# TennisBowling/grandine

Measured on AMD Instinct MI355X. Metric: verified BLS signature sets/sec (whole node), higher is better.
Workload: dtype u32 (exact 381-bit Montgomery: 12 x 32-bit limbs; 14 x 28-bit limbs in the Miller products and the square-root exponentiations); 1 GPU; C2: 16 independent batches of 4096 single-pubkey sets per GPU per step, each its own random-scalar multi_verify (segments of one submission); config=C2, streams_in_flight=2, parallelism=1 GPU

## Files before the change

grandine_amd/csrc/bls_dfp_tables.h:

```cpp
#pragma once
#include <stdint.h>
namespace gbls { namespace dfp {
constexpr uint64_t X_ABS = 0xd201000000010000ull;
constexpr int W12D_ZERO = 72, W12D_NSLOT = 73;
__constant__ uint8_t W12D_PRE[54][8] = {
  {0, 12, 12, 12, 12, 12, 12, 12},
  {1, 12, 12, 12, 12, 12, 12, 12},
  {0, 1, 12, 12, 12, 12, 12, 12},
  {2, 12, 12, 12, 12, 12, 12, 12},
  {3, 12, 12, 12, 12, 12, 12, 12},
  {2, 3, 12, 12, 12, 12, 12, 12},
  {4, 12, 12, 12, 12, 12, 12, 12},
  {5, 12, 12, 12, 12, 12, 12, 12},
  {4, 5, 12, 12, 12, 12, 12, 12},
  {2, 4, 12, 12, 12, 12, 12, 12},
  {3, 5, 12, 12, 12, 12, 12, 12},
  {2, 3, 4, 5, 12, 12, 12, 12},
  {0, 2, 12, 12, 12, 12, 12, 12},
  {1, 3, 12, 12, 12, 12, 12, 12},
  {0, 1, 2, 3, 12, 12, 12, 12},
  {0, 4, 12, 12, 12, 12, 12, 12},
  {1, 5, 12, 12, 12, 12, 12, 12},
  {0, 1, 4, 5, 12, 12, 12, 12},
  {6, 12, 12, 12, 12, 12, 12, 12},
// ... 266 lines not shown
};
__constant__ uint32_t K_FROB2[6][16] = {
  {0xdba9366u, 0xb7fde37u, 0x25bc342u, 0x894e275u, 0x1e97784u, 0x9dc1f5bu, 0x2b2b91bu, 0xfcafb87u, 0x06f497du, 0xa9b0bb2u, 0x137cc89u, 0xe399594u, 0xd9d20d7u, 0x000411cu, 0x0000000u, 0x0000000u},
  {0x9f59d6au, 0xdf5d035u, 0x06879dbu, 0x20871fdu, 0x40009cbu, 0xafc0735u, 0xb30b1b0u, 0x540793cu, 0xe51b64cu, 0xbe10100u, 0xc7f3381u, 0xc5133bcu, 0x9a653e5u, 0x00126bau, 0x0000000u, 0x0000000u},
  {0xc3b0a04u, 0x275f1fdu, 0xe0cb699u, 0x9738f87u, 0x2169246u, 0x11fe7dau, 0x87df895u, 0x5757db5u, 0xde26cceu, 0x145f54eu, 0xb4766f8u, 0xe179e28u, 0xc09330du, 0x000e59du, 0x0000000u, 0x0000000u},
  {0x2451745u, 0x47021c8u, 0x1a43c77u, 0x76b08a0u, 0x43aa727u, 0x0334bb4u, 0xcb477b7u, 0xf6d55a4u, 0x4080206u, 0xa1fc1c4u, 0xa6fe9b9u, 0x0300f1du, 0x44d18a8u, 0x0015ef4u, 0x0000000u, 0x0000000u},
  {0x60a0d41u, 0x1fa2fcau, 0x39785deu, 0xdf77918u, 0x22414e0u, 0xf1363dau, 0x4367f21u, 0x9f7d7efu, 0x6259538u, 0x8d9cc75u, 0xf2882c1u, 0x21870f4u, 0x843e59au, 0x0007956u, 0x0000000u, 0x0000000u},
  {0x3c4a0a7u, 0xd7a0e02u, 0x5f34920u, 0x68c5b8du, 0x40d8c65u, 0x8ef8335u, 0x6e9383du, 0x9c2d376u, 0x694deb6u, 0x374d827u, 0x0604f4bu, 0x0520689u, 0x5e10672u, 0x000ba73u, 0x0000000u, 0x0000000u},
};
constexpr uint32_t K_P_U[16] = {0xfffaaabu, 0xfefffffu, 0x3ffffb9u, 0xfffeb15u, 0x6241eabu, 0xa0f6b0fu, 0xf6730d2u, 0xf38512bu, 0x4774b84u, 0x4bacd76u, 0xba7b643u, 0xe69a4b1u, 0x1ea397fu, 0x001a011u, 0x0000000u, 0x0000000u};
constexpr uint32_t K_PINV_U[16] = {0xffcfffdu, 0xf3fffcfu, 0x113e889u, 0xdb92d9du, 0xb48286au, 0xf0c8e30u, 0xc16ef2eu, 0x8eb2db4u, 0x9ecca0eu, 0x68cf581u, 0x316fee2u, 0xfc9468bu, 0x106feaau, 0xa0ceb06u, 0x27f7e27u, 0xd0d7f87u};
__constant__ uint32_t K_P[16] = {0x0fffaaabu, 0x0fefffffu, 0x03ffffb9u, 0x0fffeb15u, 0x06241eabu, 0x0a0f6b0fu, 0x0f6730d2u, 0x0f38512bu, 0x04774b84u, 0x04bacd76u, 0x0ba7b643u, 0x0e69a4b1u, 0x01ea397fu, 0x0001a011u, 0x00000000u, 0x00000000u};
__constant__ uint32_t K_CIN[16] = {0x062b6c9du, 0x07d3988au, 0x0aff4e96u, 0x0383fa8eu, 0x08464532u, 0x08703310u, 0x0f823830u, 0x0d396d7cu, 0x05efebb5u, 0x04e16bc1u, 0x07cd07eeu, 0x056c4fabu, 0x0d3a884eu, 0x00002cb5u, 0x00000000u, 0x00000000u};
__constant__ uint32_t K_COUT[16] = {0x0002fffdu, 0x00900000u, 0x0c000276u, 0x0000bc40u, 0x08baebf4u, 0x05753c75u, 0x055f4898u, 0x07052574u, 0x07ce5853u, 0x056ec6d7u, 0x071a97a2u, 0x0e4935c0u, 0x0ec3fa80u, 0x00015f65u, 0x00000000u, 0x00000000u};
__constant__ uint32_t K_ONE[16] = {0x0dba9366u, 0x0b7fde37u, 0x025bc342u, 0x0894e275u, 0x01e97784u, 0x09dc1f5bu, 0x02b2b91bu, 0x0fcafb87u, 0x006f497du, 0x0a9b0bb2u, 0x0137cc89u, 0x0e399594u, 0x0d9d20d7u, 0x0000411cu, 0x00000000u, 0x00000000u};
__constant__ uint32_t K_BIAS_R1[16] = {0x7ffd5558u, 0x7f7ffff8u, 0x7ffffdc8u, 0x7fff58a2u, 0x7120f558u, 0x707b5874u, 0x7b39868eu, 0x79c28958u, 0x73ba5c20u, 0x75d66babu, 0x7d3db213u, 0x734d2586u, 0x7f51cbf8u, 0x000d0081u, 0x00000000u, 0x00000000u};
__constant__ uint32_t K_BIAS_R2[16] = {0x3ff55560u, 0x3dfffffcu, 0x3ffff73cu, 0x3ffd62a4u, 0x3483d57cu, 0x31ed61e9u, 0x3ce61a51u, 0x370a257bu, 0x3ee9709bu, 0x3759aec5u, 0x34f6c866u, 0x3d349634u, 0x3d472ff9u, 0x00340220u, 0x00000000u, 0x00000000u};
__constant__ uint32_t K_BIAS_NEG[16] = {0x2fd55580u, 0x27fffffdu, 0x2fffdcfdu, 0x2ff58a9du, 0x220f55fdu, 0x27b587afu, 0x2398694eu, 0x2c2895f9u, 0x2ba5c277u, 0x2d66bb21u, 0x23db21a3u, 0x24d258dbu, 0x251cbff1u, 0x00d0088du, 0x00000000u, 0x00000000u};
__constant__ uint32_t K_BIAS_SQ[16] = {0x5eaaac00u, 0x5ffffffau, 0x5ffee7f6u, 0x5fac54fau, 0x507aaffau, 0x5dac3d84u, 0x5cc34a7eu, 0x5144afd4u, 0x5d2e13c9u, 0x5b35d918u, 0x5ed90d29u, 0x5692c6e4u, 0x58e5ff95u, 0x06804475u, 0x00000000u, 0x00000000u};
__constant__ uint32_t K_BIAS_GY[16] = {0x3f555600u, 0x3ffffffcu, 0x3fff73fau, 0x3fd62a7cu, 0x383d57fcu, 0x3ed61ec1u, 0x3e61a53eu, 0x30a257e9u, 0x3e9709e4u, 0x359aec8bu, 0x3f6c8694u, 0x33496371u, 0x3472ffcau, 0x0340223au, 0x00000000u, 0x00000000u};
__constant__ uint32_t K_BIAS_GS[16] = {0x4eaaac00u, 0x4ffffffbu, 0x4ffee7f7u, 0x4fac54fbu, 0x407aaffbu, 0x4dac3d85u, 0x4cc34a7fu, 0x4144afd5u, 0x4d2e13cau, 0x4b35d919u, 0x4ed90d2au, 0x4692c6e5u, 0x48e5ff96u, 0x06804476u, 0x00000000u, 0x00000000u};
__constant__ uint32_t K_INVFIX[16] = {0x06b0f5bau, 0x079ca4b9u, 0x0d0e7df7u, 0x02e27c00u, 0x0b969102u, 0x005b1d88u, 0x0f3b945du, 0x0051805fu, 0x02710831u, 0x0ea54e57u, 0x095e4bd3u, 0x055e4a8du, 0x042b7a0fu, 0x0000e87du, 0x00000000u, 0x00000000u};
__constant__ uint32_t K_PSI_CX1[16] = {0x03c4a0a7u, 0x0d7a0e02u, 0x05f34920u, 0x068c5b8du, 0x040d8c65u, 0x08ef8335u, 0x06e9383du, 0x09c2d376u, 0x0694deb6u, 0x0374d827u, 0x00604f4bu, 0x00520689u, 0x05e10672u, 0x0000ba73u, 0x00000000u, 0x00000000u};
__constant__ uint32_t K_PSI_CY0[16] = {0x04c22d67u, 0x0947f37bu, 0x0853ec71u, 0x002485e1u, 0x015b9b2au, 0x0b1268c5u, 0x0b62e6e6u, 0x045fb220u, 0x04dd1ca9u, 0x04fcbb2cu, 0x00af4fc4u, 0x05fd3770u, 0x0475233bu, 0x0000faafu, 0x00000000u, 0x00000000u};
__constant__ uint32_t K_PSI_CY1[16] = {0x0b3d7d44u, 0x06a80c84u, 0x0bac1348u, 0x0fdb6533u, 0x04c88381u, 0x0efd024au, 0x040449ebu, 0x0ad89f0bu, 0x0f9a2edbu, 0x0fbe1249u, 0x0af8667eu, 0x086c6d41u, 0x0d751644u, 0x0000a561u, 0x00000000u, 0x00000000u};
__constant__ uint32_t K_PSI2_CX[16] = {0x060a0d41u, 0x01fa2fcau, 0x039785deu, 0x0df77918u, 0x022414e0u, 0x0f1363dau, 0x04367f21u, 0x09f7d7efu, 0x06259538u, 0x08d9cc75u, 0x0f2882c1u, 0x021870f4u, 0x0843e59au, 0x00007956u, 0x00000000u, 0x00000000u};
__constant__ uint32_t K_PSI2_CY[16] = {0x02451745u, 0x047021c8u, 0x01a43c77u, 0x076b08a0u, 0x043aa727u, 0x00334bb4u, 0x0cb477b7u, 0x0f6d55a4u, 0x04080206u, 0x0a1fc1c4u, 0x0a6fe9b9u, 0x00300f1du, 0x044d18a8u, 0x00015ef4u, 0x00000000u, 0x00000000u};
__constant__ uint32_t K_BIASK[10][16] = {
  {0x2fff5556u, 0x2fdffffdu, 0x27ffff71u, 0x2fffd628u, 0x2c483d55u, 0x241ed61cu, 0x2ece61a3u, 0x2e70a255u, 0x28ee9707u, 0x29759aeau, 0x274f6c84u, 0x2cd34961u, 0x23d472fdu, 0x00034020u, 0x00000000u, 0x00000000u},
  {0x2ffeaaacu, 0x2fbffffdu, 0x2ffffee5u, 0x2fffac52u, 0x28907aadu, 0x283dac3bu, 0x2d9cc348u, 0x2ce144adu, 0x21dd2e11u, 0x22eb35d7u, 0x2e9ed90bu, 0x29a692c4u, 0x27a8e5fdu, 0x00068042u, 0x00000000u, 0x00000000u},
// ... 11 lines not shown
```

grandine_amd/csrc/bls_w4.h:

```cpp
#pragma once
#include "bls_curve.h"
#include "bls_dfp.h"
#include "bls_pairing.h"

namespace gbls {
namespace w4 {

struct Ctx {
  dfp::Tabs t;
  uint32_t r;
  uint32_t bias[10];
  uint32_t one;
};
__device__ __forceinline__ void init(Ctx &c) {
  dfp::load_tabs(c.t);
  c.r = (threadIdx.x >> 4) & 3;
#pragma unroll
  for (int k = 0; k < 10; k++) c.bias[k] = dfp::K_BIASK[k][c.t.j];
  c.one = dfp::konst(dfp::K_ONE);
}

__device__ __forceinline__ void exclusive_simd() { asm volatile("" ::: "v255", "a255"); }
constexpr uint32_t kExclusiveMaxWaves = 512;

// ... 87 lines not shown
  f2 x, y;
};

__device__ __forceinline__ uint32_t repack(const fp &a, uint32_t j) {
  uint32_t v = 0;
#pragma unroll
  for (int i = 0; i < 14; i++) {
    const int bit = 28 * i, k = bit >> 5, sh = bit & 31;
    uint64_t pair = a.l[k];
    if (k + 1 < 12) pair |= (uint64_t)a.l[k + 1] << 32;
    const uint32_t limb = (uint32_t)(pair >> sh) & dfp::M28;
    v = j == (uint32_t)i ? limb : v;
  }
  return v;
}
__device__ __forceinline__ void load(const Ctx &c, J &o, const g2j &p) {
  const uint32_t cin = dfp::konst(dfp::K_CIN);
  uint32_t v[6] = {repack(p.x.c0, c.t.j), repack(p.x.c1, c.t.j), repack(p.y.c0, c.t.j),
                   repack(p.y.c1, c.t.j), repack(p.z.c0, c.t.j), repack(p.z.c1, c.t.j)};
  mul4(c, o.x.c0, o.x.c1, o.y.c0, o.y.c1, v[0], cin, v[1], cin, v[2], cin, v[3], cin);
  uint32_t d0, d1;
  mul4(c, o.z.c0, o.z.c1, d0, d1, v[4], cin, v[5], cin, v[4], cin, v[5], cin);
}
__device__ __forceinline__ void load(const Ctx &c, A2 &o, const g2a &p) {
  const uint32_t cin = dfp::konst(dfp::K_CIN);
  mul4(c, o.x.c0, o.x.c1, o.y.c0, o.y.c1, repack(p.x.c0, c.t.j), cin, repack(p.x.c1, c.t.j), cin,
       repack(p.y.c0, c.t.j), cin, repack(p.y.c1, c.t.j), cin);
}
__device__ __forceinline__ void store4(const Ctx &c, uint32_t v0, uint32_t v1, uint32_t v2,
                                       uint32_t v3, uint32_t *w0, uint32_t *w1, uint32_t *w2,
                                       uint32_t *w3) {
  uint32_t *w = c.r == 0 ? w0 : (c.r == 1 ? w1 : (c.r == 2 ? w2 : w3));
  dfp::to_words(w, sel(c, v0, v1, v2, v3), c.t);
}

__device__ __forceinline__ void store_jac(const Ctx &c, g2j *o, const J &p) {
  store4(c, p.x.c0, p.x.c1, p.y.c0, p.y.c1, o->x.c0.l, o->x.c1.l, o->y.c0.l, o->y.c1.l);
  const uint32_t w = dfp::word_of(sel(c, p.z.c0, p.z.c1, p.z.c0, p.z.c1), c.t);
// ... 485 lines not shown
```

grandine_amd/csrc/gbls_capi.hip:

```cpp
#include <hip/hip_runtime.h>

#include <algorithm>
#include <atomic>
#include <condition_variable>
#include <cstdio>
#include <cstdlib>
#include <cstring>
#include <memory>
#include <chrono>
#include <cerrno>
#include <sys/random.h>
#include <mutex>
#include <shared_mutex>
#include <vector>

#include "../../include/grandine_bls_gpu.h"
#include "../../include/grandine_bls_gpu_committees.h"
#include "../../include/grandine_bls_gpu_msgcache.h"
#include "../../include/grandine_bls_gpu_msgcache_checks.h"
#include "../../include/grandine_bls_gpu_bits.h"
#include "../../include/grandine_bls_gpu_each.h"
#include "../../include/grandine_bls_gpu_spans.h"
#include "../../include/grandine_bls_gpu_local.h"
#include "../../include/grandine_bls_gpu_fold.h"
// ... 882 lines not shown
      !c.ensure(c.V0, ML_EVENTS * mt.v0_n * sizeof(fp12)) ||
      !c.ensure(c.V1, ML_EVENTS * mt.v1_n * sizeof(fp12)) ||
      (g_ml_r28 && !c.ensure(c.V28, (size_t)ML_EVENTS * 168 * 4 * mt.ngroup)) ||
      (g_ml_r28 && mt.ngp && !c.ensure(c.Pc, (size_t)36 * 4 * mt.ncol)) ||
      !c.ensure(c.hparts, 4 * 64 * sizeof(fp12)))
    return false;
  if (!c.upload_staged(c.tab, tab.data(), tab.size() * 4, st)) return false;
  const uint32_t N = (uint32_t)n, NP = (uint32_t)np, NS = (uint32_t)nseg, NQ = (uint32_t)nq, NM = (uint32_t)nm;
  const uint32_t n_store = mcp ? (uint32_t)mcp->store_pair.size() : 0;
  const uint32_t n_copy = mcp ? mcp->ncopy : 0;
  const bool hash_msgs = !mcp || NM;
  if (pl && trace_dedup())
    fprintf(stderr, "gbls dedup: sets=%zu segments=%zu groups=%zu pairs=%zu%s\n", n, nseg, nq, np,
            mcp ? " (line cache)" : "");
  g2j *sj = nullptr;
  if (!msm && !single && !sliced && X == 1 && nseg <= kW4Max) {
    if (!c.ensure(c.Sj, nseg * sizeof(g2j) + 16)) return false;
    sj = c.Sj.as<g2j>();
  }
  const uint32_t *T = c.tab.as<uint32_t>();
  const LineCols lc{mt.ngp ? T + mt.col_off : nullptr, mt.ncol};
  c.line_col = lc.col;
  c.line_ncol = lc.ncol;
  g2j *gpart = c.gpart.as<g2j>();
  int32_t *gpart_err = reinterpret_cast<int32_t *>(gpart + nchunks);
  HIPCHK(hipEventRecord(c.ev_fork, st));
  HIPCHK(hipStreamWaitEvent(side1, c.ev_fork, 0));
  HIPCHK(hipStreamWaitEvent(side2, c.ev_fork, 0));
  if (mcp && NQ - n_copy > NM) {
    StageTimer t(S_LC_LOAD, st);
    launch_linecache_load(st, c.mc_tab->dev, T + mc_ix_at, NM, NQ - n_copy - NM, lc, c.lines.as<uint32_t>());
  }
// ... 18 lines not shown
    if (sig_groupcheck) {
      HIPCHK(hipMemcpyAsync(c.pre2.p, c.sig_st, (size_t)N * 4, hipMemcpyDeviceToDevice, side2));
      launch_g2_check(side2, sigs, N, c.pre2.as<int32_t>(), 1);
      pre2 = c.pre2.as<int32_t>();
    }
    c.sig_c = nullptr;
    c.sig_st = nullptr;
  } else if (sig_groupcheck) {
    launch_g2_check(side2, sigs, N, c.pre2.as<int32_t>(), 0);
    pre2 = c.pre2.as<int32_t>();
  }
  if (msm) {
    HIPCHK(hipStreamWaitEvent(side2, c.ev_pks, 0));
    StageTimer t(S_MSM, side2);
    launch_msm(side2, mp, c.msm.as<uint8_t>(), sigs, rands, pks, pre, pre2, N, T + segoff_at,
               empty_is_error, c.H.as<g2a>(), c.P.as<g1s>(), seg_err, NQ);
  } else if (!single) {
    StageTimer t(S_G2MUL, side2);
    launch_mv_g2mul(side2, sigs, rands, N, c.R.as<g2j>());
  }
  if (!msm) {
    StageTimer t(S_G2SUM, side2);
    if (single) {
      HIPCHK(hipStreamWaitEvent(side2, c.ev_pks, 0));
      launch_single_S(side2, sigs, pks, pre, pre2, N, c.P.as<g1s>(), c.H.as<g2a>(), seg_err,
                      grouped ? c.ng1.as<g1a>() : nullptr);
      if (grouped)
        launch_mv_g1mul(side2, c.ng1.as<g1a>(), grp_r, N, c.P.as<g1s>() + N);
    } else {
      launch_g2sum(side2, c.R.as<g2j>(), T + chunk_off, (uint32_t)nchunks, T + segchunk_off,
                   T + segoff_at, NS, N, pks, rands, pre, pre2, empty_is_error, gpart, gpart_err,
                   c.P.as<g1s>(), c.H.as<g2a>(), seg_err, sj, c.ev_pks, NQ);
    }
  }
  const bool lines_s_main = msm && !sliced && g.lines_s_main;
  if (!lines_s_main) {
    StageTimer t(S_LINES_S, side2);
    if (!sj || !launch_lines_jac(side2, sj, 1, NQ, NS, lc, c.lines.as<uint32_t>()))
      launch_lines(side2, c.H.as<g2a>(), NQ, (uint32_t)(nseg * X), lc, 0, EC, c.Ts.as<g2h>(),
                   c.lines.as<uint32_t>(), g.lines_s_lane);
  }
  const bool jac_h = !sliced && NM <= kW4Max;
  if (hash_msgs) set_side_lines(c, st, NM, jac_h, lc, EC);
  HIPCHK(hipEventRecord(c.ev_side1, side1));
  HIPCHK(hipEventRecord(c.ev_side2, side2));
  if (n_store && n_copy) {
    const uint32_t *ix = T + mc_ix_at + (NQ - NM);
    {
      StageTimer t(S_LC_STORE, st);
      launch_linecache_store(st, c.mc_tab->dev, ix, ix + n_store, n_store, lc, c.lines.as<uint32_t>());
    }
    StageTimer t(S_LC_LOAD, st);
    launch_linecache_load(st, c.mc_tab->dev, T + mc_ix_at + (NQ - NM - n_copy), NQ - n_copy, n_copy, lc,
// ... 2276 lines not shown
```

grandine_amd/csrc/gbls_common.h:

```cpp
#pragma once
#include <hip/hip_runtime.h>

#include "bls_hash.h"
#include "bls_pairing.h"

namespace gbls {

constexpr int WG = 64;
constexpr int WGR = 256;
constexpr uint32_t NONE = 0xffffffffu;
constexpr uint32_t kLaneRegimeSets = 8192;
constexpr uint32_t kRowRegimeMax = 6144;
#ifndef GBLS_W4_MAX
#define GBLS_W4_MAX 1024
#endif
constexpr uint32_t kW4Max = GBLS_W4_MAX;
constexpr uint32_t kRowClearMax = 2048;
extern uint32_t g_row_clear_max;
extern uint32_t g_ml_r28;
constexpr uint32_t kMsmChunk = 16;
constexpr uint32_t kMsmChunkSmall = 4;
constexpr int kMsmFoldLevels = 3;
constexpr uint32_t kMsmFold = 1u << kMsmFoldLevels;
extern uint32_t g_msm_k;
// ... 79 lines not shown
  uint32_t nb;
  uint32_t max_chunks;
  uint32_t K;
  uint32_t max_folds;
  bool tree;
  uint32_t extra;
  bool r28;
  size_t o_cnt, o_start, o_cur, o_cstart, o_fstart[kMsmFoldLevels], o_list, o_chunk, o_t0, o_a0, o_t1, o_a1,
      o_sig28, bytes;
};
constexpr uint32_t kMsmMinPerSeg = 2048;
MsmPlan msm_plan(uint32_t n, uint32_t nseg);
void launch_msm(hipStream_t st, const MsmPlan &p, uint8_t *ws, const g2a *sigs,
                const uint64_t *rands, const g1a *pks, const int32_t *pre, const int32_t *pre2,
                uint32_t n, const uint32_t *seg_off, int empty_is_error, g2a *H, g1s *P,
                int32_t *seg_err, uint32_t xbase = NONE);

struct LineCols {
  const uint32_t *col;
  uint32_t ncol;
};
void launch_lines(hipStream_t st, const g2a *H, uint32_t first, uint32_t count, LineCols lc,
                  int e0, int e1, g2h *Ts, uint32_t *lines, bool lane = false);
bool launch_lines_jac(hipStream_t st, const g2j *Qj, uint32_t stride, uint32_t first, uint32_t count,
                      LineCols lc, uint32_t *lines);

void launch_linecache_load(hipStream_t st, const uint32_t *tab, const uint32_t *slot, uint32_t first,
                           uint32_t count, LineCols lc, uint32_t *lines);
void launch_linecache_store(hipStream_t st, uint32_t *tab, const uint32_t *pairs, const uint32_t *slot,
                            uint32_t count, LineCols lc, const uint32_t *lines);

// ... 22 lines not shown
```

grandine_amd/csrc/k_miller.hip:

```cpp
#include "bls_wave12.h"
#include "bls_w12d.h"
#include "bls_field28.h"
#include "gbls_common.h"

namespace gbls {

__device__ __forceinline__ uint32_t ml_col(const LineCols &lc, uint32_t ngp, uint32_t g, uint32_t j,
                                           uint32_t pair) {
  return ngp ? j * ngp + g : (lc.col ? lc.col[pair] : pair);
}
__device__ __forceinline__ void ml_eval(sp034 &s, const uint32_t *L, uint32_t ncol, uint32_t col,
                                        const g1s *P, uint32_t pair, int e) {
  fp2 L0, L2, L3;
  line_get(L, ncol, col, e, L0, L2, L3);
  g1s Pp = P[pair];
  line_eval_s(s, L0, L2, L3, Pp);
}

__device__ __forceinline__ uint32_t xcd_work_index(uint32_t b, uint32_t nwg) {
  const uint32_t xcd = b % 8, q = nwg / 8, r = nwg % 8;
  return (xcd < r ? xcd * (q + 1) : r * (q + 1) + (xcd - r) * q) + b / 8;
}
__global__ void __launch_bounds__(WG) k_ml_group(const uint32_t *L, LineCols lc, uint32_t ngp, const g1s *P,
                                                 const uint32_t *plist, const uint32_t *grp,
// ... 412 lines not shown
    fp_mul(o.y, p.y, inv);
    fp_one(o.c);
  }
  const uint32_t *w = reinterpret_cast<const uint32_t *>(&o);
#pragma unroll
  for (int i = 0; i < 36; i++) Pc[(size_t)i * ncol + c] = w[i];
}
void launch_ml_pcols(hipStream_t st, const g1s *P, const uint32_t *col, uint32_t np, uint32_t ncol,
                     uint32_t *Pc, bool normalize) {
  if (!np) return;
  if (normalize)
    k_ml_pcols<true><<<nblk(np), WG, 0, st>>>(P, col, np, ncol, Pc);
  else
    k_ml_pcols<false><<<nblk(np), WG, 0, st>>>(P, col, np, ncol, Pc);
}
void launch_ml_group(hipStream_t st, const uint32_t *lines, LineCols lc, uint32_t ngp, const g1s *P,
                     const uint32_t *Pc, const uint32_t *plist, const uint32_t *groups, uint32_t ngroup, int e0,
                     int e1, fp12 *V0, uint32_t *V28, bool pcn) {
  dim3 grid(nblk(ngroup), e1 - e0);
  if (!ngroup || e1 <= e0) return;
  const dim3 grid1(nblk(ngroup) * (uint32_t)(e1 - e0));
  if (g_ml_r28 && V28) {
    if (g_ml_dma)
      k_ml_group28<true, false><<<grid1, WG, 0, st>>>(lines, lc, ngp, P, Pc, plist, groups, ngroup, e0, e1 - e0, (int)g_ml_xcd, V28);
    else if (g_ml_kara && pcn)
      k_ml_group28<false, false, true, true><<<grid1, WG, 0, st>>>(lines, lc, ngp, P, Pc, plist, groups, ngroup, e0, e1 - e0, (int)g_ml_xcd, V28);
    else if (g_ml_kara)
      k_ml_group28<false, false, true><<<grid1, WG, 0, st>>>(lines, lc, ngp, P, Pc, plist, groups, ngroup, e0, e1 - e0, (int)g_ml_xcd, V28);
    else if (g_ml_prefetch && pcn)
      k_ml_group28<false, true, false, true><<<grid1, WG, 0, st>>>(lines, lc, ngp, P, Pc, plist, groups, ngroup, e0, e1 - e0, (int)g_ml_xcd, V28);
    else if (g_ml_prefetch)
      k_ml_group28<false, true><<<grid1, WG, 0, st>>>(lines, lc, ngp, P, Pc, plist, groups, ngroup, e0, e1 - e0, (int)g_ml_xcd, V28);
    else if (pcn)
      k_ml_group28<false, false, false, true><<<grid1, WG, 0, st>>>(lines, lc, ngp, P, Pc, plist, groups, ngroup, e0, e1 - e0, (int)g_ml_xcd, V28);
    else
      k_ml_group28<false, false><<<grid1, WG, 0, st>>>(lines, lc, ngp, P, Pc, plist, groups, ngroup, e0, e1 - e0, (int)g_ml_xcd, V28);
    const uint32_t nvals = ngroup * (uint32_t)(e1 - e0);
    k_ml_pack28<<<nblk((size_t)nvals * 12), WG, 0, st>>>(V28, ngroup, e0, nvals, V0);
    return;
  }
  k_ml_group<<<grid1, WG, 0, st>>>(lines, lc, ngp, P, plist, groups, ngroup, e0, e1 - e0, (int)g_ml_xcd, V0);
}
void launch_ml_reduce(hipStream_t st, const fp12 *Vin, uint32_t nin, const uint32_t *red,
                      uint32_t nout, fp12 *Vout) {
  dim3 grid(nout, ML_EVENTS);
  if (nout) k_ml_reduce<<<grid, 64, 0, st>>>(Vin, nin, red, nout, Vout);
}
struct HornerParts {
  int n;
  int b[8];
};
constexpr HornerParts kHornerParts4 = {4, {0, 7, 18, 36, 68, 68, 68, 68}};
constexpr HornerParts kHornerParts1 = {1, {0, 68, 68, 68, 68, 68, 68, 68}};

__global__ void __launch_bounds__(w12d::THREADS) k_ml_horner_d(const fp12 *V, uint32_t nseg,
                                                               fp12 *out, const uint32_t *lim,
// ... 57 lines not shown
```

grandine_amd/csrc/k_msm.hip:

```cpp
#include "gbls_common.h"
#include "bls_gang.h"
#include "bls_curve28.h"

namespace gbls {


__device__ __forceinline__ int msm_digit(uint64_t k, int w, int c, uint32_t &carry) {
  uint64_t raw = (c * w < 64) ? (k >> (c * w)) & ((1ull << c) - 1) : 0;
  int d = (int)raw + (int)carry;
  if (d > (1 << (c - 1))) {
    d -= 1 << c;
    carry = 1;
  } else {
    carry = 0;
  }
  return d;
}
__device__ __forceinline__ uint32_t msm_segment(const uint32_t *seg_off, uint32_t nseg, uint32_t i) {
  uint32_t lo = 0, hi = nseg;
  while (hi - lo > 1) {
    uint32_t mid = (lo + hi) >> 1;
    if (seg_off[mid] <= i)
      lo = mid;
    else
// ... 207 lines not shown
    r28::g2j_load12(s, chunk[c0]);
    for (uint32_t w = c0 + kMsmFold; w < c1; w += kMsmFold) {
      r28::g2j_load12(y, chunk[w]);
      jac_add(s, s, y);
    }
    r28::g2j_out(x, s);
  } else {
    x = chunk[c0];
    for (uint32_t w = c0 + kMsmFold; w < c1; w += kMsmFold) {
      g2j y = chunk[w];
      jac_add(x, x, y);
    }
  }
}

__device__ __forceinline__ void msm_weight(g1s &o, const uint32_t *table, uint32_t k) {
#pragma unroll
  for (int i = 0; i < 12; i++) {
    o.x.l[i] = table[24 * k + i];
    o.y.l[i] = table[24 * k + 12 + i];
  }
  fp_one(o.c);
}

template <bool R28>
__global__ void __launch_bounds__(WG) k_msm_pairs(const g2j *chunk, const uint32_t *cstart,
                                                  uint32_t nb, uint32_t per_seg, uint32_t n,
                                                  const uint32_t *seg_off, int empty_is_error,
                                                  g1s *P, g2a *H, int32_t *seg_err) {
  uint32_t t = blockIdx.x * WG + threadIdx.x;
  if (t >= nb) return;
  uint32_t s = t / per_seg, k = t % per_seg;
  g2j x;
  msm_bucket_sum<R28>(x, chunk, cstart, t);
  g2a a;
  jac_to_aff(a, x);
  g1s w;
  msm_weight(w, k::MSM_W5, k);
  P[n + t] = w;
  H[n + t] = a;
  if (k == 0 && empty_is_error && seg_off[s + 1] == seg_off[s]) atomicOr(&seg_err[s], 1);
}

template <bool R28>
__global__ void __launch_bounds__(WG) k_msm_bucket(const g2j *chunk, const uint32_t *cstart,
                                                   uint32_t nb, g2j *T, g2j *A) {
  uint32_t b = blockIdx.x * WG + threadIdx.x;
  if (b >= nb) return;
  g2j x, inf;
  msm_bucket_sum<R28>(x, chunk, cstart, b);
  jac_set_inf(inf);
  T[b] = x;
  A[b] = inf;
}

__global__ void __launch_bounds__(WG) k_msm_tree(const g2j *Tin, const g2j *Ain, uint32_t groups,
                                                 uint32_t m, int l, g2j *Tout, g2j *Aout) {
  uint32_t t = blockIdx.x * WG + threadIdx.x;
// ... 23 lines not shown
  jac_to_aff(o, a);
  g1s g;
  msm_weight(g, k::MSM_W13, w);
  P[n + t] = g;
  H[n + t] = o;
  if (w == 0 && empty_is_error && seg_off[s + 1] == seg_off[s]) atomicOr(&seg_err[s], 1);
}

MsmPlan msm_plan(uint32_t n, uint32_t nseg) {
  uint32_t avg = nseg ? n / nseg : n;
  MsmPlan p;
  p.nseg = nseg;
  p.c = avg >= (1u << 16) ? 13 : 5;
  p.W = 65 / p.c;
  p.tree = p.c == 13;
  p.extra = p.tree ? (uint32_t)p.W : ((uint32_t)p.W << (p.c - 1));
  p.nb = nseg * ((uint32_t)p.W << (p.c - 1));
  p.K = g_msm_k ? g_msm_k : (avg < 4096 ? kMsmChunkSmall : kMsmChunk);
  p.max_chunks = (uint32_t)(((uint64_t)p.W * n + p.K - 1) / p.K) + p.nb;
  p.max_folds = p.max_chunks / 2 + p.nb;
  size_t o = 0;
  auto take = [&](size_t bytes) {
    size_t at = o;
    o += (bytes + 255) & ~(size_t)255;
    return at;
  };
  p.o_cnt = take(p.nb * 4);
  p.o_start = take((p.nb + 1) * 4);
  p.o_cur = take(p.nb * 4);
  p.o_cstart = take((p.nb + 1) * 4);
  for (int l = 0; l < kMsmFoldLevels; l++) p.o_fstart[l] = take((p.nb + 1) * 4);
// ... 1 lines not shown
  p.o_chunk = take((size_t)p.max_chunks * sizeof(g2j));
  const size_t tn = p.tree ? p.nb : 0;
  p.o_t0 = take(tn * sizeof(g2j));
  p.o_a0 = take(tn * sizeof(g2j));
  p.o_t1 = take((tn / 2 + 1) * sizeof(g2j));
  p.o_a1 = take((tn / 2 + 1) * sizeof(g2j));
  p.r28 = g_msm_r28 != 0;
  p.o_sig28 = take(p.r28 ? (size_t)n * sizeof(g2a) : 0);
  p.bytes = o;
  return p;
}

void launch_msm(hipStream_t st, const MsmPlan &p, uint8_t *ws, const g2a *sigs,
                const uint64_t *rands, const g1a *pks, const int32_t *pre, const int32_t *pre2,
                uint32_t n, const uint32_t *seg_off, int empty_is_error, g2a *H, g1s *P,
                int32_t *seg_err, uint32_t xbase) {
  const uint32_t xb = xbase == NONE ? n : xbase;
  uint32_t *cnt = reinterpret_cast<uint32_t *>(ws + p.o_cnt);
  uint32_t *start = reinterpret_cast<uint32_t *>(ws + p.o_start);
  uint32_t *cur = reinterpret_cast<uint32_t *>(ws + p.o_cur);
  uint32_t *cstart = reinterpret_cast<uint32_t *>(ws + p.o_cstart);
  MsmFoldStarts fs;
  for (int l = 0; l < kMsmFoldLevels; l++) fs.l[l] = reinterpret_cast<uint32_t *>(ws + p.o_fstart[l]);
  uint32_t *list = reinterpret_cast<uint32_t *>(ws + p.o_list);
  g2j *chunk = reinterpret_cast<g2j *>(ws + p.o_chunk);
  (void)hipMemsetAsync(cnt, 0, p.nb * 4, st);
  (void)hipMemsetAsync(seg_err, 0, p.nseg * 4, st);
  g2a *sig28 = p.r28 ? reinterpret_cast<g2a *>(ws + p.o_sig28) : nullptr;
  k_msm_count<<<nblk(n, WGR), WGR, 0, st>>>(sigs, rands, n, seg_off, p.nseg, p.c, p.W, pks, pre,
                                            pre2, cnt, seg_err, sig28);
  k_msm_scan<<<1, 1024, 0, st>>>(cnt, p.nb, p.K, start, cur, cstart, fs);
// ... 1 lines not shown
                                              list);
  if (p.r28)
    k_msm_chunk28<<<nblk(p.max_chunks), WG, 0, st>>>(sig28, list, start, cstart, p.nb, p.max_chunks,
                                                     p.K, chunk);
  else
    k_msm_chunk<<<nblk(p.max_chunks), WG, 0, st>>>(sigs, list, start, cstart, p.nb, p.max_chunks,
                                                   p.K, chunk);
  for (int l = 0; l < kMsmFoldLevels; l++) {
    const uint32_t mp = (p.max_folds >> l) + p.nb;
    if (p.r28)
      k_msm_fold28<<<nblk(mp), WG, 0, st>>>(cstart, fs.l[l], p.nb, mp, l, chunk);
    else
      k_msm_fold<<<nblk(mp), WG, 0, st>>>(cstart, fs.l[l], p.nb, mp, l, chunk);
  }
  if (!p.tree) {
    if (p.r28)
      k_msm_pairs<true><<<nblk(p.nb), WG, 0, st>>>(chunk, cstart, p.nb, p.extra, xb, seg_off,
                                                   empty_is_error, P, H, seg_err);
    else
      k_msm_pairs<false><<<nblk(p.nb), WG, 0, st>>>(chunk, cstart, p.nb, p.extra, xb, seg_off,
                                                    empty_is_error, P, H, seg_err);
    return;
  }
  g2j *T[2] = {reinterpret_cast<g2j *>(ws + p.o_t0), reinterpret_cast<g2j *>(ws + p.o_t1)};
  g2j *A[2] = {reinterpret_cast<g2j *>(ws + p.o_a0), reinterpret_cast<g2j *>(ws + p.o_a1)};
  if (p.r28)
    k_msm_bucket<true><<<nblk(p.nb), WG, 0, st>>>(chunk, cstart, p.nb, T[0], A[0]);
  else
    k_msm_bucket<false><<<nblk(p.nb), WG, 0, st>>>(chunk, cstart, p.nb, T[0], A[0]);
  int src = 0;
  const uint32_t B = 1u << (p.c - 1), groups = p.nseg * (uint32_t)p.W;
  for (int l = 0; (1u << (l + 1)) <= B; l++) {
    uint32_t m = B >> (l + 1);
    k_msm_tree<<<nblk((size_t)groups * m), WG, 0, st>>>(T[src], A[src], groups, m, l, T[1 - src],
                                                         A[1 - src]);
    src = 1 - src;
// ... 7 lines not shown
```

Baseline: 4.802 million sets/s.

## Reduce MSM buckets per window on device with wave-parallel w4 kernel

Replaces the per-bucket k_msm_pairs output, which emitted one affine G2 point and G1 weight per bucket for the pairing, with a w4 gang kernel that does a running-sum bucket reduction per window. Each window is then a single pairing input, which cuts the pairing count per segment by the bucket count. Results can be stored in Jacobian form to feed the Jacobian line path directly. It also adds an R28 load constant and gates the ML XCD remap on grid size. The cost is extra G2 adds and doublings in a serial per-window kernel with limited parallelism.

```diff
diff --git a/grandine_amd/csrc/bls_dfp_tables.h b/grandine_amd/csrc/bls_dfp_tables.h
--- a/grandine_amd/csrc/bls_dfp_tables.h
+++ b/grandine_amd/csrc/bls_dfp_tables.h
@@ -304,6 +304,7 @@
 __constant__ uint32_t K_CIN[16] = {0x062b6c9du, 0x07d3988au, 0x0aff4e96u, 0x0383fa8eu, 0x08464532u, 0x08703310u, 0x0f823830u, 0x0d396d7cu, 0x05efebb5u, 0x04e16bc1u, 0x07cd07eeu, 0x056c4fabu, 0x0d3a884eu, 0x00002cb5u, 0x00000000u, 0x00000000u};
 __constant__ uint32_t K_COUT[16] = {0x0002fffdu, 0x00900000u, 0x0c000276u, 0x0000bc40u, 0x08baebf4u, 0x05753c75u, 0x055f4898u, 0x07052574u, 0x07ce5853u, 0x056ec6d7u, 0x071a97a2u, 0x0e4935c0u, 0x0ec3fa80u, 0x00015f65u, 0x00000000u, 0x00000000u};
 __constant__ uint32_t K_ONE[16] = {0x0dba9366u, 0x0b7fde37u, 0x025bc342u, 0x0894e275u, 0x01e97784u, 0x09dc1f5bu, 0x02b2b91bu, 0x0fcafb87u, 0x006f497du, 0x0a9b0bb2u, 0x0137cc89u, 0x0e399594u, 0x0d9d20d7u, 0x0000411cu, 0x00000000u, 0x00000000u};
+__constant__ uint32_t K_CIN28[16] = {0x08a61dc2u, 0x06054398u, 0x0f5eff43u, 0x0be380a0u, 0x08740f2eu, 0x0ec4e858u, 0x08770909u, 0x000d3e6du, 0x0b2d0b04u, 0x0b56cc53u, 0x0225a938u, 0x0ca457b0u, 0x073bbdbdu, 0x000042cfu, 0x00000000u, 0x00000000u};
 __constant__ uint32_t K_BIAS_R1[16] = {0x7ffd5558u, 0x7f7ffff8u, 0x7ffffdc8u, 0x7fff58a2u, 0x7120f558u, 0x707b5874u, 0x7b39868eu, 0x79c28958u, 0x73ba5c20u, 0x75d66babu, 0x7d3db213u, 0x734d2586u, 0x7f51cbf8u, 0x000d0081u, 0x00000000u, 0x00000000u};
 __constant__ uint32_t K_BIAS_R2[16] = {0x3ff55560u, 0x3dfffffcu, 0x3ffff73cu, 0x3ffd62a4u, 0x3483d57cu, 0x31ed61e9u, 0x3ce61a51u, 0x370a257bu, 0x3ee9709bu, 0x3759aec5u, 0x34f6c866u, 0x3d349634u, 0x3d472ff9u, 0x00340220u, 0x00000000u, 0x00000000u};
 __constant__ uint32_t K_BIAS_NEG[16] = {0x2fd55580u, 0x27fffffdu, 0x2fffdcfdu, 0x2ff58a9du, 0x220f55fdu, 0x27b587afu, 0x2398694eu, 0x2c2895f9u, 0x2ba5c277u, 0x2d66bb21u, 0x23db21a3u, 0x24d258dbu, 0x251cbff1u, 0x00d0088du, 0x00000000u, 0x00000000u};
diff --git a/grandine_amd/csrc/bls_w4.h b/grandine_amd/csrc/bls_w4.h
--- a/grandine_amd/csrc/bls_w4.h
+++ b/grandine_amd/csrc/bls_w4.h
@@ -125,14 +125,15 @@
   }
   return v;
 }
-__device__ __forceinline__ void load(const Ctx &c, J &o, const g2j &p) {
-  const uint32_t cin = dfp::konst(dfp::K_CIN);
+__device__ __forceinline__ void load(const Ctx &c, J &o, const g2j &p, uint32_t cin) {
   uint32_t v[6] = {repack(p.x.c0, c.t.j), repack(p.x.c1, c.t.j), repack(p.y.c0, c.t.j),
                    repack(p.y.c1, c.t.j), repack(p.z.c0, c.t.j), repack(p.z.c1, c.t.j)};
   mul4(c, o.x.c0, o.x.c1, o.y.c0, o.y.c1, v[0], cin, v[1], cin, v[2], cin, v[3], cin);
   uint32_t d0, d1;
   mul4(c, o.z.c0, o.z.c1, d0, d1, v[4], cin, v[5], cin, v[4], cin, v[5], cin);
 }
+__device__ __forceinline__ void load(const Ctx &c, J &o, const g2j &p) { load(c, o, p, dfp::konst(dfp::K_CIN)); }
+__device__ __forceinline__ void load28(const Ctx &c, J &o, const g2j &p) { load(c, o, p, dfp::konst(dfp::K_CIN28)); }
 __device__ __forceinline__ void load(const Ctx &c, A2 &o, const g2a &p) {
   const uint32_t cin = dfp::konst(dfp::K_CIN);
   mul4(c, o.x.c0, o.x.c1, o.y.c0, o.y.c1, repack(p.x.c0, c.t.j), cin, repack(p.x.c1, c.t.j), cin,
diff --git a/grandine_amd/csrc/gbls_capi.hip b/grandine_amd/csrc/gbls_capi.hip
--- a/grandine_amd/csrc/gbls_capi.hip
+++ b/grandine_amd/csrc/gbls_capi.hip
@@ -920,8 +920,9 @@
     fprintf(stderr, "gbls dedup: sets=%zu segments=%zu groups=%zu pairs=%zu%s\n", n, nseg, nq, np,
             mcp ? " (line cache)" : "");
   g2j *sj = nullptr;
-  if (!msm && !single && !sliced && X == 1 && nseg <= kW4Max) {
-    if (!c.ensure(c.Sj, nseg * sizeof(g2j) + 16)) return false;
+  const bool msm_jac = msm && !mp.tree && !g.lines_s_main;
+  if ((msm ? msm_jac : !single && X == 1) && !sliced && nseg * X <= kW4Max) {
+    if (!c.ensure(c.Sj, nseg * X * sizeof(g2j) + 16)) return false;
     sj = c.Sj.as<g2j>();
   }
   const uint32_t *T = c.tab.as<uint32_t>();
@@ -970,7 +971,7 @@
     HIPCHK(hipStreamWaitEvent(side2, c.ev_pks, 0));
     StageTimer t(S_MSM, side2);
     launch_msm(side2, mp, c.msm.as<uint8_t>(), sigs, rands, pks, pre, pre2, N, T + segoff_at,
-               empty_is_error, c.H.as<g2a>(), c.P.as<g1s>(), seg_err, NQ);
+               empty_is_error, c.H.as<g2a>(), c.P.as<g1s>(), seg_err, NQ, sj);
   } else if (!single) {
     StageTimer t(S_G2MUL, side2);
     launch_mv_g2mul(side2, sigs, rands, N, c.R.as<g2j>());
@@ -992,7 +993,7 @@
   const bool lines_s_main = msm && !sliced && g.lines_s_main;
   if (!lines_s_main) {
     StageTimer t(S_LINES_S, side2);
-    if (!sj || !launch_lines_jac(side2, sj, 1, NQ, NS, lc, c.lines.as<uint32_t>()))
+    if (!sj || !launch_lines_jac(side2, sj, 1, NQ, (uint32_t)(nseg * X), lc, c.lines.as<uint32_t>()))
       launch_lines(side2, c.H.as<g2a>(), NQ, (uint32_t)(nseg * X), lc, 0, EC, c.Ts.as<g2h>(),
                    c.lines.as<uint32_t>(), g.lines_s_lane);
   }
diff --git a/grandine_amd/csrc/gbls_common.h b/grandine_amd/csrc/gbls_common.h
--- a/grandine_amd/csrc/gbls_common.h
+++ b/grandine_amd/csrc/gbls_common.h
@@ -117,7 +117,7 @@
 void launch_msm(hipStream_t st, const MsmPlan &p, uint8_t *ws, const g2a *sigs,
                 const uint64_t *rands, const g1a *pks, const int32_t *pre, const int32_t *pre2,
                 uint32_t n, const uint32_t *seg_off, int empty_is_error, g2a *H, g1s *P,
-                int32_t *seg_err, uint32_t xbase = NONE);
+                int32_t *seg_err, uint32_t xbase = NONE, g2j *Sj = nullptr);
 
 struct LineCols {
   const uint32_t *col;
diff --git a/grandine_amd/csrc/k_miller.hip b/grandine_amd/csrc/k_miller.hip
--- a/grandine_amd/csrc/k_miller.hip
+++ b/grandine_amd/csrc/k_miller.hip
@@ -450,32 +450,34 @@
   else
     k_ml_pcols<false><<<nblk(np), WG, 0, st>>>(P, col, np, ncol, Pc);
 }
+constexpr uint32_t kMlXcdMinBlocks = 1536;
 void launch_ml_group(hipStream_t st, const uint32_t *lines, LineCols lc, uint32_t ngp, const g1s *P,
                      const uint32_t *Pc, const uint32_t *plist, const uint32_t *groups, uint32_t ngroup, int e0,
                      int e1, fp12 *V0, uint32_t *V28, bool pcn) {
   dim3 grid(nblk(ngroup), e1 - e0);
   if (!ngroup || e1 <= e0) return;
   const dim3 grid1(nblk(ngroup) * (uint32_t)(e1 - e0));
+  const int xcd = g_ml_xcd && grid1.x > kMlXcdMinBlocks ? (int)g_ml_xcd : 0;
   if (g_ml_r28 && V28) {
     if (g_ml_dma)
-      k_ml_group28<true, false><<<grid1, WG, 0, st>>>(lines, lc, ngp, P, Pc, plist, groups, ngroup, e0, e1 - e0, (int)g_ml_xcd, V28);
+      k_ml_group28<true, false><<<grid1, WG, 0, st>>>(lines, lc, ngp, P, Pc, plist, groups, ngroup, e0, e1 - e0, xcd, V28);
     else if (g_ml_kara && pcn)
-      k_ml_group28<false, false, true, true><<<grid1, WG, 0, st>>>(lines, lc, ngp, P, Pc, plist, groups, ngroup, e0, e1 - e0, (int)g_ml_xcd, V28);
+      k_ml_group28<false, false, true, true><<<grid1, WG, 0, st>>>(lines, lc, ngp, P, Pc, plist, groups, ngroup, e0, e1 - e0, xcd, V28);
     else if (g_ml_kara)
-      k_ml_group28<false, false, true><<<grid1, WG, 0, st>>>(lines, lc, ngp, P, Pc, plist, groups, ngroup, e0, e1 - e0, (int)g_ml_xcd, V28);
+      k_ml_group28<false, false, true><<<grid1, WG, 0, st>>>(lines, lc, ngp, P, Pc, plist, groups, ngroup, e0, e1 - e0, xcd, V28);
     else if (g_ml_prefetch && pcn)
-      k_ml_group28<false, true, false, true><<<grid1, WG, 0, st>>>(lines, lc, ngp, P, Pc, plist, groups, ngroup, e0, e1 - e0, (int)g_ml_xcd, V28);
+      k_ml_group28<false, true, false, true><<<grid1, WG, 0, st>>>(lines, lc, ngp, P, Pc, plist, groups, ngroup, e0, e1 - e0, xcd, V28);
     else if (g_ml_prefetch)
-      k_ml_group28<false, true><<<grid1, WG, 0, st>>>(lines, lc, ngp, P, Pc, plist, groups, ngroup, e0, e1 - e0, (int)g_ml_xcd, V28);
+      k_ml_group28<false, true><<<grid1, WG, 0, st>>>(lines, lc, ngp, P, Pc, plist, groups, ngroup, e0, e1 - e0, xcd, V28);
     else if (pcn)
-      k_ml_group28<false, false, false, true><<<grid1, WG, 0, st>>>(lines, lc, ngp, P, Pc, plist, groups, ngroup, e0, e1 - e0, (int)g_ml_xcd, V28);
+      k_ml_group28<false, false, false, true><<<grid1, WG, 0, st>>>(lines, lc, ngp, P, Pc, plist, groups, ngroup, e0, e1 - e0, xcd, V28);
     else
-      k_ml_group28<false, false><<<grid1, WG, 0, st>>>(lines, lc, ngp, P, Pc, plist, groups, ngroup, e0, e1 - e0, (int)g_ml_xcd, V28);
+      k_ml_group28<false, false><<<grid1, WG, 0, st>>>(lines, lc, ngp, P, Pc, plist, groups, ngroup, e0, e1 - e0, xcd, V28);
     const uint32_t nvals = ngroup * (uint32_t)(e1 - e0);
     k_ml_pack28<<<nblk((size_t)nvals * 12), WG, 0, st>>>(V28, ngroup, e0, nvals, V0);
     return;
   }
-  k_ml_group<<<grid1, WG, 0, st>>>(lines, lc, ngp, P, plist, groups, ngroup, e0, e1 - e0, (int)g_ml_xcd, V0);
+  k_ml_group<<<grid1, WG, 0, st>>>(lines, lc, ngp, P, plist, groups, ngroup, e0, e1 - e0, xcd, V0);
 }
 void launch_ml_reduce(hipStream_t st, const fp12 *Vin, uint32_t nin, const uint32_t *red,
                       uint32_t nout, fp12 *Vout) {
diff --git a/grandine_amd/csrc/k_msm.h b/grandine_amd/csrc/k_msm.h
--- /dev/null
+++ b/grandine_amd/csrc/k_msm.h
@@ -0,0 +1,18 @@
+#pragma once
+#include "gbls_common.h"
+
+namespace gbls {
+
+__device__ __forceinline__ void msm_weight(g1s &o, const uint32_t *table, uint32_t k) {
+#pragma unroll
+  for (int i = 0; i < 12; i++) {
+    o.x.l[i] = table[24 * k + i];
+    o.y.l[i] = table[24 * k + 12 + i];
+  }
+  fp_one(o.c);
+}
+void launch_msm_windows_w4(hipStream_t st, const g2j *chunk, const uint32_t *cstart, uint32_t nwin, uint32_t W,
+                           bool r28, uint32_t xb, const uint32_t *seg_off, int empty_is_error, g1s *P, g2a *H,
+                           int32_t *seg_err, g2j *Sj);
+
+}
diff --git a/grandine_amd/csrc/k_msm.hip b/grandine_amd/csrc/k_msm.hip
--- a/grandine_amd/csrc/k_msm.hip
+++ b/grandine_amd/csrc/k_msm.hip
@@ -1,4 +1,5 @@
 #include "gbls_common.h"
+#include "k_msm.h"
 #include "bls_gang.h"
 #include "bls_curve28.h"
 
@@ -245,34 +246,6 @@
   }
 }
 
-__device__ __forceinline__ void msm_weight(g1s &o, const uint32_t *table, uint32_t k) {
-#pragma unroll
-  for (int i = 0; i < 12; i++) {
-    o.x.l[i] = table[24 * k + i];
-    o.y.l[i] = table[24 * k + 12 + i];
-  }
-  fp_one(o.c);
-}
-
-template <bool R28>
-__global__ void __launch_bounds__(WG) k_msm_pairs(const g2j *chunk, const uint32_t *cstart,
-                                                  uint32_t nb, uint32_t per_seg, uint32_t n,
-                                                  const uint32_t *seg_off, int empty_is_error,
-                                                  g1s *P, g2a *H, int32_t *seg_err) {
-  uint32_t t = blockIdx.x * WG + threadIdx.x;
-  if (t >= nb) return;
-  uint32_t s = t / per_seg, k = t % per_seg;
-  g2j x;
-  msm_bucket_sum<R28>(x, chunk, cstart, t);
-  g2a a;
-  jac_to_aff(a, x);
-  g1s w;
-  msm_weight(w, k::MSM_W5, k);
-  P[n + t] = w;
-  H[n + t] = a;
-  if (k == 0 && empty_is_error && seg_off[s + 1] == seg_off[s]) atomicOr(&seg_err[s], 1);
-}
-
 template <bool R28>
 __global__ void __launch_bounds__(WG) k_msm_bucket(const g2j *chunk, const uint32_t *cstart,
                                                    uint32_t nb, g2j *T, g2j *A) {
@@ -326,7 +299,7 @@
   p.c = avg >= (1u << 16) ? 13 : 5;
   p.W = 65 / p.c;
   p.tree = p.c == 13;
-  p.extra = p.tree ? (uint32_t)p.W : ((uint32_t)p.W << (p.c - 1));
+  p.extra = (uint32_t)p.W;
   p.nb = nseg * ((uint32_t)p.W << (p.c - 1));
   p.K = g_msm_k ? g_msm_k : (avg < 4096 ? kMsmChunkSmall : kMsmChunk);
   p.max_chunks = (uint32_t)(((uint64_t)p.W * n + p.K - 1) / p.K) + p.nb;
@@ -358,7 +331,7 @@
 void launch_msm(hipStream_t st, const MsmPlan &p, uint8_t *ws, const g2a *sigs,
                 const uint64_t *rands, const g1a *pks, const int32_t *pre, const int32_t *pre2,
                 uint32_t n, const uint32_t *seg_off, int empty_is_error, g2a *H, g1s *P,
-                int32_t *seg_err, uint32_t xbase) {
+                int32_t *seg_err, uint32_t xbase, g2j *Sj) {
   const uint32_t xb = xbase == NONE ? n : xbase;
   uint32_t *cnt = reinterpret_cast<uint32_t *>(ws + p.o_cnt);
   uint32_t *start = reinterpret_cast<uint32_t *>(ws + p.o_start);
@@ -390,12 +363,8 @@
       k_msm_fold<<<nblk(mp), WG, 0, st>>>(cstart, fs.l[l], p.nb, mp, l, chunk);
   }
   if (!p.tree) {
-    if (p.r28)
-      k_msm_pairs<true><<<nblk(p.nb), WG, 0, st>>>(chunk, cstart, p.nb, p.extra, xb, seg_off,
-                                                   empty_is_error, P, H, seg_err);
-    else
-      k_msm_pairs<false><<<nblk(p.nb), WG, 0, st>>>(chunk, cstart, p.nb, p.extra, xb, seg_off,
-                                                    empty_is_error, P, H, seg_err);
+    launch_msm_windows_w4(st, chunk, cstart, p.nseg * (uint32_t)p.W, (uint32_t)p.W, p.r28, xb, seg_off,
+                          empty_is_error, P, H, seg_err, Sj);
     return;
   }
   g2j *T[2] = {reinterpret_cast<g2j *>(ws + p.o_t0), reinterpret_cast<g2j *>(ws + p.o_t1)};
diff --git a/grandine_amd/csrc/k_msm_w4.hip b/grandine_amd/csrc/k_msm_w4.hip
--- /dev/null
+++ b/grandine_amd/csrc/k_msm_w4.hip
@@ -0,0 +1,89 @@
+#include "gbls_common.h"
+#include "k_msm.h"
+#include "bls_w4.h"
+
+namespace gbls {
+
+constexpr int kMsmW4Waves = 2;
+constexpr int kMsmW4Buckets = 16;
+template <bool X, bool R28>
+__global__ void __launch_bounds__(64 * kMsmW4Waves) k_msm_windows_w4(const g2j *chunk, const uint32_t *cstart,
+                                                                    uint32_t nwin, uint32_t W, uint32_t xb,
+                                                                    const uint32_t *seg_off, int empty_is_error,
+                                                                    g1s *P, g2a *H, int32_t *seg_err, g2j *Sj) {
+  if constexpr (X) w4::exclusive_simd();
+  constexpr int NW = kMsmW4Waves, BW = kMsmW4Buckets / NW;
+  static_assert(NW >= 1 && (NW & (NW - 1)) == 0 && NW <= kMsmW4Buckets, "a power of two of waves");
+  __shared__ uint32_t sh[NW > 1 ? NW / 2 : 1][6 * 64];
+  const uint32_t t = blockIdx.x;
+  if (t >= nwin) return;
+  const uint32_t v = threadIdx.x >> 6, lane = threadIdx.x & 63;
+  w4::Ctx c;
+  w4::init(c);
+  w4::J T, A;
+  w4::set_inf(c, T);
+  w4::set_inf(c, A);
+  const uint32_t lo = t * kMsmW4Buckets + v * BW;
+  for (uint32_t b = lo + BW; b-- > lo;) {
+    const uint32_t c0 = cstart[b], c1 = cstart[b + 1];
+    for (uint32_t q = c0; q < c1; q += kMsmFold) {
+      w4::J x;
+      if constexpr (R28)
+        w4::load28(c, x, chunk[q]);
+      else
+        w4::load(c, x, chunk[q]);
+      w4::add(c, T, T, x);
+    }
+    w4::add(c, A, A, T);
+  }
+  if (v) {
+    const uint32_t m = v * BW;
+    w4::J D = T;
+    for (int bit = 30 - __clz((int)m); bit >= 0; bit--) {
+      w4::dbl(c, D, D);
+      if ((m >> bit) & 1) w4::add(c, D, D, T);
+    }
+    w4::add(c, A, A, D);
+  }
+  for (uint32_t width = NW / 2; width > 0; width >>= 1) {
+    __syncthreads();
+    if (v >= width && v < 2 * width) {
+      uint32_t *d = sh[v - width] + lane;
+      const uint32_t s[6] = {A.x.c0, A.x.c1, A.y.c0, A.y.c1, A.z.c0, A.z.c1};
+#pragma unroll
+      for (int k = 0; k < 6; k++) d[64 * k] = s[k];
+    }
+    __syncthreads();
+    if (v < width) {
+      const uint32_t *d = sh[v] + lane;
+      w4::J o;
+      o.x = {d[0], d[64]};
+      o.y = {d[128], d[192]};
+      o.z = {d[256], d[320]};
+      w4::add(c, A, A, o);
+    }
+  }
+  if (v != 0) return;
+  if (Sj)
+    w4::store_jac(c, Sj + t, A);
+  else
+    w4::store_affine(c, H + xb + t, A);
+  if (threadIdx.x == 0) {
+    const uint32_t s = t / W, w = t % W;
+    g1s g;
+    msm_weight(g, k::MSM_W5, kMsmW4Buckets * w);
+    P[xb + t] = g;
+    if (w == 0 && empty_is_error && seg_off[s + 1] == seg_off[s]) atomicOr(&seg_err[s], 1);
+  }
+}
+
+void launch_msm_windows_w4(hipStream_t st, const g2j *chunk, const uint32_t *cstart, uint32_t nwin, uint32_t W,
+                           bool r28, uint32_t xb, const uint32_t *seg_off, int empty_is_error, g1s *P, g2a *H,
+                           int32_t *seg_err, g2j *Sj) {
+  const bool x = nwin * kMsmW4Waves <= w4::kExclusiveMaxWaves;
+  auto k = r28 ? (x ? k_msm_windows_w4<true, true> : k_msm_windows_w4<false, true>)
+               : (x ? k_msm_windows_w4<true, false> : k_msm_windows_w4<false, false>);
+  k<<<nwin, 64 * kMsmW4Waves, 0, st>>>(chunk, cstart, nwin, W, xb, seg_off, empty_is_error, P, H, seg_err, Sj);
+}
+
+}
```

New measurement: 4.894 million sets/s, median of 6. +1.9%, better.
